# YiZhiXiaoGuLI/xerus

Measured on AMD Instinct MI355X. Metric: GFLOP/s on TT contraction + TT-round sweep time, order-10 rank-256, higher is better.
Workload: dtype f64; 1 GPU; TT order-10 n=20 rank-256: <x,y> + x.round(256) per step; order=10, mode_size=20, rank=256, parallelism=replicas x1

## Files before the change

### include/xerus_amd.h

```cpp
#ifndef XERUS_AMD_H
#define XERUS_AMD_H

#include <stddef.h>
#include <stdint.h>

#ifdef __cplusplus
extern "C" {
#endif

typedef struct xrs_handle_s* xrs_handle_t;

#define XRS_OK 0
#define XRS_EINVAL (-1)
#define XRS_ENOMEM (-2)
#define XRS_EHIP (-3)
#define XRS_ENUMERIC 1

int xrs_create(xrs_handle_t* handle, int device);
int xrs_destroy(xrs_handle_t handle);
int xrs_set_stream(xrs_handle_t handle, void* hip_stream);
void* xrs_get_stream(xrs_handle_t handle);
int xrs_synchronize(xrs_handle_t handle);
const char* xrs_last_error(void);
const char* xrs_version(void);

int xrs_malloc(xrs_handle_t handle, void** ptr, size_t bytes);
int xrs_free(xrs_handle_t handle, void* ptr);
size_t xrs_pool_bytes(xrs_handle_t handle);
int xrs_upload(xrs_handle_t handle, double* dst_dev, const double* src_host, size_t n);
int xrs_download(xrs_handle_t handle, double* dst_host, const double* src_dev, size_t n);
int xrs_memset_zero(xrs_handle_t handle, double* dst_dev, size_t n);
int xrs_copy(xrs_handle_t handle, double* dst_dev, const double* src_dev, size_t n);

int xrs_nrm2(xrs_handle_t handle, double* result, const double* x, size_t n);
int xrs_dot(xrs_handle_t handle, double* result, const double* x, const double* y, size_t n);
int xrs_asum(xrs_handle_t handle, double* result, const double* x, size_t n);
int xrs_scal(xrs_handle_t handle, double* x, double alpha, size_t n);
int xrs_axpy(xrs_handle_t handle, double* y, double alpha, const double* x, size_t n);
int xrs_scale_rows(xrs_handle_t handle, double* X, const double* s, size_t m, size_t n);

int xrs_gemm(xrs_handle_t handle, double* C, size_t M, size_t N, double alpha,
             const double* A, size_t lda, int transA, size_t K,
             const double* B, size_t ldb, int transB);

int xrs_gemm_batched(xrs_handle_t handle, size_t count, double* const* C, size_t M, size_t N, double alpha,
                     const double* const* A, size_t lda, int transA, size_t K,
                     const double* const* B, size_t ldb, int transB);

int xrs_gemm_sym(xrs_handle_t handle, double* C, size_t N, double alpha,
                 const double* A, size_t lda, int transA, size_t K,
                 const double* B, size_t ldb, int transB);

int xrs_gemm_forms(xrs_handle_t handle, size_t count, double* const* C, size_t M, size_t N, double alpha,
                   const double* const* A, size_t lda, int transA, size_t K,
                   const double* const* B, size_t ldb, int transB, int sym, int tri);

int xrs_gemm_f32(xrs_handle_t handle, float* C, size_t M, size_t N, float alpha,
                 const float* A, size_t lda, int transA, size_t K,
                 const float* B, size_t ldb, int transB);

int xrs_permute(xrs_handle_t handle, double* out, const double* in, size_t ndim,
                const size_t* dims, const size_t* shuffle);

int xrs_qc(xrs_handle_t handle, double* Q, double* C, size_t* rank, const double* A, size_t m, size_t n);
int xrs_cq(xrs_handle_t handle, double* C, double* Q, size_t* rank, const double* A, size_t m, size_t n);
int xrs_qr(xrs_handle_t handle, double* Q, double* R, const double* A, size_t m, size_t n);
int xrs_rq(xrs_handle_t handle, double* R, double* Q, const double* A, size_t m, size_t n);
int xrs_svd(xrs_handle_t handle, double* U, double* S, double* Vt, const double* A, size_t m, size_t n);
int xrs_svd_batched(xrs_handle_t handle, double* U, double* S, double* Vt, int* status,
                    const double* A, size_t batch, size_t m, size_t n);
int xrs_svd_batched_fits(size_t m, size_t n);
int xrs_solve(xrs_handle_t handle, double* X, const double* A, size_t m, size_t n, const double* B, size_t p);
int xrs_solve_least_squares(xrs_handle_t handle, double* X, const double* A, size_t m, size_t n, const double* B, size_t p);
int xrs_svd_rows_vt(xrs_handle_t handle, double* S, double* Vt, int* sweeps, const double* A, size_t p, size_t q, int kernel);
int xrs_sym_tridiag(xrs_handle_t handle, double* d, double* e, const double* A, size_t n);
int xrs_sym_eig_top(xrs_handle_t handle, double* lam, double* Ut, int* status, const double* A, size_t n, size_t kk);


int xrs_tt_move_core(xrs_handle_t handle, size_t d, const size_t* n, size_t* r, double** cores,
                     int canonicalized, size_t core_position, size_t position, int keep_rank);
int xrs_tt_round(xrs_handle_t handle, size_t d, const size_t* n, size_t* r, double** cores,
                 int canonicalized, size_t core_position, const size_t* max_ranks, double eps);
int xrs_tt_soft_threshold(xrs_handle_t handle, size_t d, const size_t* n, size_t* r, double** cores,
                          int canonicalized, size_t core_position, const double* taus);
int xrs_tt_entrywise_product(xrs_handle_t handle, size_t d, const size_t* ext, const size_t* ra, const double* const* A,
                             const size_t* rb, const double* const* B, double alpha, double** out);
int xrs_tt_entrywise_square(xrs_handle_t handle, size_t d, const size_t* ext, const size_t* r, const double* const* A,
                            double alpha, double** out, size_t* r_out);
// ... 60 lines not shown

int xrs_philox_words(xrs_handle_t handle, uint32_t* out, size_t s, size_t q, uint64_t seed, uint32_t stream);
int xrs_gaussian_matrix(xrs_handle_t handle, double* G, size_t s, size_t m, uint64_t seed, uint32_t stream);
#define XRS_SKETCH_FUSED 1
#define XRS_SKETCH_MATERIALISED 2
int xrs_sketch_gaussian(xrs_handle_t handle, double* Y, size_t s, const double* A, size_t m, size_t n, uint64_t seed,
                        uint32_t stream, int route);
int xrs_sketch_last_route(xrs_handle_t handle);


int xrs_als_local_apply(xrs_handle_t handle, double* y, const double* x, size_t rl, size_t n, size_t rr, size_t pl,
                        size_t pr, const double* L, const double* A, const double* R, int normal);
#define XRS_CG_CONVERGED 0
#define XRS_CG_MAX_ITER 1
#define XRS_CG_BREAKDOWN 2
int xrs_als_local_cg(xrs_handle_t handle, double* x, const double* b, size_t rl, size_t n, size_t rr, size_t pl,
                     size_t pr, const double* L, const double* A, const double* R, int normal, double tol,
                     size_t max_iter, size_t check_every, size_t* iters, double* relres, int* status);

#define XRS_EIG_CONVERGED 0
#define XRS_EIG_MAX_ITER 1
#define XRS_EIG_BREAKDOWN 2
int xrs_als_local_eig(xrs_handle_t handle, double* x, size_t rl, size_t n, size_t rr, size_t pl, size_t pr,
                      const double* L, const double* A, const double* R, double tol, size_t max_iter, size_t check_every,
                      double* theta, size_t* iters, double* relres, int* status);
int xrs_geneig_lowest(int k, const double* G, const double* H, double* theta, double* c);

#define XRS_KFAM_GEMM 1u
#define XRS_KFAM_PERMUTE 2u
#define XRS_KFAM_QR 4u
#define XRS_KFAM_SVD 8u
#define XRS_KFAM_ELEMWISE 16u
#define XRS_KFAM_SPLITK 32u
int xrs_prof_begin(xrs_handle_t handle, uint32_t family_mask);
int xrs_prof_end(xrs_handle_t handle, size_t* launches, double* total_ms, double* flops, double* bytes);

#ifdef __cplusplus
}
#endif
#endif
```

### xerus_amd/capi.py

```python
from __future__ import annotations

import ctypes as C
import os
from typing import Sequence

import numpy as np

_HERE = os.path.dirname(os.path.abspath(__file__))
LIB_PATH = os.environ.get("XRS_LIB_PATH") or os.path.join(_HERE, "libxerus_amd.so")

_SZ = C.c_size_t
_DP = C.c_void_p

SIGNATURES = {
    "xrs_create": (C.c_int, [C.POINTER(_DP), C.c_int]),
    "xrs_destroy": (C.c_int, [_DP]),
    "xrs_set_stream": (C.c_int, [_DP, _DP]),
    "xrs_get_stream": (_DP, [_DP]),
    "xrs_synchronize": (C.c_int, [_DP]),
    "xrs_last_error": (C.c_char_p, []),
    "xrs_version": (C.c_char_p, []),
    "xrs_malloc": (C.c_int, [_DP, C.POINTER(_DP), _SZ]),
    "xrs_free": (C.c_int, [_DP, _DP]),
    "xrs_pool_bytes": (_SZ, [_DP]),
    "xrs_upload": (C.c_int, [_DP, _DP, _DP, _SZ]),
    "xrs_download": (C.c_int, [_DP, _DP, _DP, _SZ]),
    "xrs_memset_zero": (C.c_int, [_DP, _DP, _SZ]),
    "xrs_copy": (C.c_int, [_DP, _DP, _DP, _SZ]),
    "xrs_nrm2": (C.c_int, [_DP, C.POINTER(C.c_double), _DP, _SZ]),
    "xrs_dot": (C.c_int, [_DP, C.POINTER(C.c_double), _DP, _DP, _SZ]),
    "xrs_asum": (C.c_int, [_DP, C.POINTER(C.c_double), _DP, _SZ]),
    "xrs_scal": (C.c_int, [_DP, _DP, C.c_double, _SZ]),
    "xrs_axpy": (C.c_int, [_DP, _DP, C.c_double, _DP, _SZ]),
    "xrs_scale_rows": (C.c_int, [_DP, _DP, _DP, _SZ, _SZ]),
    "xrs_gemm": (C.c_int, [_DP, _DP, _SZ, _SZ, C.c_double, _DP, _SZ, C.c_int, _SZ, _DP, _SZ, C.c_int]),
    "xrs_gemm_f32": (C.c_int, [_DP, _DP, _SZ, _SZ, C.c_float, _DP, _SZ, C.c_int, _SZ, _DP, _SZ, C.c_int]),
    "xrs_gemm_sym": (C.c_int,[_DP, _DP, _SZ, C.c_double, _DP, _SZ, C.c_int, _SZ, _DP, _SZ, C.c_int]),
    "xrs_gemm_batched": (C.c_int, [_DP, _SZ, C.POINTER(_DP), _SZ, _SZ, C.c_double, C.POINTER(_DP), _SZ, C.c_int, _SZ,
                                   C.POINTER(_DP), _SZ, C.c_int]),
    "xrs_gemm_forms": (C.c_int, [_DP, _SZ, C.POINTER(_DP), _SZ, _SZ, C.c_double, C.POINTER(_DP), _SZ, C.c_int, _SZ,
                                 C.POINTER(_DP), _SZ, C.c_int, C.c_int, C.c_int]),
    "xrs_permute": (C.c_int, [_DP, _DP, _DP, _SZ, C.POINTER(_SZ), C.POINTER(_SZ)]),
    "xrs_qc": (C.c_int, [_DP, _DP, _DP, C.POINTER(_SZ), _DP, _SZ, _SZ]),
    "xrs_cq": (C.c_int, [_DP, _DP, _DP, C.POINTER(_SZ), _DP, _SZ, _SZ]),
    "xrs_qr": (C.c_int, [_DP, _DP, _DP, _DP, _SZ, _SZ]),
    "xrs_rq": (C.c_int, [_DP, _DP, _DP, _DP, _SZ, _SZ]),
    "xrs_svd": (C.c_int, [_DP, _DP, _DP, _DP, _DP, _SZ, _SZ]),
    "xrs_svd_batched": (C.c_int, [_DP, _DP, _DP, _DP, C.POINTER(C.c_int), _DP, _SZ, _SZ, _SZ]),
    "xrs_svd_batched_fits": (C.c_int, [_SZ, _SZ]),
    "xrs_solve": (C.c_int, [_DP, _DP, _DP, _SZ, _SZ, _DP, _SZ]),
    "xrs_solve_least_squares": (C.c_int, [_DP, _DP, _DP, _SZ, _SZ, _DP, _SZ]),
    "xrs_svd_rows_vt": (C.c_int, [_DP, _DP, _DP, C.POINTER(C.c_int), _DP, _SZ, _SZ, C.c_int]),
    "xrs_sym_eig_top": (C.c_int, [_DP, _DP, _DP, C.POINTER(C.c_int), _DP, _SZ, _SZ]),
    "xrs_sym_tridiag": (C.c_int, [_DP, _DP, _DP, _DP, _SZ]),
    "xrs_tt_entrywise_product": (C.c_int, [_DP, _SZ, C.POINTER(_SZ), C.POINTER(_SZ), C.POINTER(_DP), C.POINTER(_SZ), C.POINTER(_DP),
                                           C.c_double, C.POINTER(_DP)]),
    "xrs_tt_entrywise_square": (C.c_int, [_DP, _SZ, C.POINTER(_SZ), C.POINTER(_SZ), C.POINTER(_DP), C.c_double, C.POINTER(_DP),
                                          C.POINTER(_SZ)]),
    "xrs_tt_rank_one_argmax": (C.c_int, [_DP, _SZ, C.POINTER(_SZ), C.POINTER(_DP), C.POINTER(_SZ)]),
    "xrs_tt_operator_apply": (C.c_int, [_DP, _SZ, C.POINTER(_SZ), C.POINTER(_SZ), C.POINTER(_SZ), C.POINTER(_SZ), C.POINTER(_DP),
                                        C.POINTER(_SZ), C.POINTER(_DP), C.c_int, C.POINTER(_DP)]),
    "xrs_tt_move_core": (C.c_int, [_DP, _SZ, C.POINTER(_SZ), C.POINTER(_SZ), C.POINTER(_DP), C.c_int, _SZ, _SZ, C.c_int]),
    "xrs_tt_round": (C.c_int, [_DP, _SZ, C.POINTER(_SZ), C.POINTER(_SZ), C.POINTER(_DP), C.c_int, _SZ,
                               C.POINTER(_SZ), C.c_double]),
    "xrs_tt_dot": (C.c_int, [_DP, C.POINTER(C.c_double), _SZ, C.POINTER(_SZ), C.POINTER(_SZ), C.POINTER(_DP),
                             C.POINTER(_SZ), C.POINTER(_DP)]),
    "xrs_tt_dot_async": (C.c_int, [_DP, _SZ, C.POINTER(_SZ), C.POINTER(_SZ), C.POINTER(_DP), C.POINTER(_SZ),
                                   C.POINTER(_DP)]),
    "xrs_tt_dot_wait": (C.c_int, [_DP, C.POINTER(C.c_double)]),
    "xrs_tt_dot_f32": (C.c_int, [_DP, C.POINTER(C.c_double), _SZ, C.POINTER(_SZ), C.POINTER(_SZ), C.POINTER(_DP),
                                 C.POINTER(_SZ), C.POINTER(_DP)]),
    "xrs_tt_round_sharded": (C.c_int, [_DP, _SZ, C.POINTER(_SZ), C.POINTER(_SZ), C.POINTER(_DP), C.POINTER(_SZ),
                                       C.c_double, _DP, _DP, C.POINTER(C.c_int)]),
    "xrs_tt_round_sharded_ex": (C.c_int, [_DP, _SZ, C.POINTER(_SZ), C.POINTER(_SZ), C.POINTER(_DP), C.POINTER(_SZ),
# ... 8 lines not shown
                                     C.POINTER(_DP), C.POINTER(_DP)]),
    "xrs_tt_last_round_path": (C.c_int, [_DP]),
    "xrs_tt_soft_threshold": (C.c_int, [_DP, _SZ, C.POINTER(_SZ), C.POINTER(_SZ), C.POINTER(_DP), C.c_int, _SZ,
                                        C.POINTER(C.c_double)]),
    "xrs_comm_unique_id": (C.c_int, [_DP]),
    "xrs_comm_create": (C.c_int, [_DP, C.c_int, C.c_int, _DP, C.POINTER(_DP)]),
    "xrs_comm_emulate": (C.c_int, [_DP, C.c_int, C.POINTER(_DP)]),
    "xrs_comm_destroy": (C.c_int, [_DP]),
    "xrs_comm_calls": (_SZ, [_DP]),
    "xrs_comm_allreduce": (C.c_int, [_DP, _DP, _SZ]),
    "xrs_comm_allgather": (C.c_int, [_DP, _DP, _DP, _SZ]),
    "xrs_tt_gather_sharded": (C.c_int, [_DP, _SZ, C.POINTER(_SZ), C.c_int, C.c_int, C.POINTER(_SZ), C.POINTER(_DP),
                                        C.POINTER(_DP), _DP, _DP]),
    "xrs_tt_shard": (C.c_int, [_DP, _SZ, C.POINTER(_SZ), C.c_int, C.c_int, C.POINTER(_SZ), C.POINTER(_DP), C.POINTER(_DP)]),
    "xrs_uq_basis": (C.c_int, [_DP, _DP, _DP, _SZ, _SZ]),
    "xrs_uq_stack_congruence": (C.c_int, [_DP, _DP, _DP, _DP, _DP, _SZ, _SZ, _SZ, _SZ]),
    "xrs_uq_quadform": (C.c_int, [_DP, C.POINTER(C.c_double), _DP, _DP, _SZ, _SZ]),
    "xrs_philox_words": (C.c_int, [_DP, _DP, _SZ, _SZ, C.c_uint64, C.c_uint32]),
    "xrs_gaussian_matrix": (C.c_int, [_DP, _DP, _SZ, _SZ, C.c_uint64, C.c_uint32]),
    "xrs_sketch_gaussian": (C.c_int, [_DP, _DP, _SZ, _DP, _SZ, _SZ, C.c_uint64, C.c_uint32, C.c_int]),
    "xrs_sketch_last_route": (C.c_int, [_DP]),
    "xrs_als_local_apply": (C.c_int, [_DP, _DP, _DP, _SZ, _SZ, _SZ, _SZ, _SZ, _DP, _DP, _DP, C.c_int]),
    "xrs_als_local_cg": (C.c_int, [_DP, _DP, _DP, _SZ, _SZ, _SZ, _SZ, _SZ, _DP, _DP, _DP, C.c_int, C.c_double, _SZ, _SZ,
                                   C.POINTER(_SZ), C.POINTER(C.c_double), C.POINTER(C.c_int)]),
    "xrs_als_local_eig": (C.c_int, [_DP, _DP, _SZ, _SZ, _SZ, _SZ, _SZ, _DP, _DP, _DP, C.c_double, _SZ, _SZ,
                                    C.POINTER(C.c_double), C.POINTER(_SZ), C.POINTER(C.c_double), C.POINTER(C.c_int)]),
    "xrs_geneig_lowest": (C.c_int, [C.c_int, C.POINTER(C.c_double), C.POINTER(C.c_double), C.POINTER(C.c_double),
                                    C.POINTER(C.c_double)]),
    "xrs_prof_begin": (C.c_int, [_DP, C.c_uint32]),
    "xrs_prof_end": (C.c_int, [_DP, C.POINTER(_SZ), C.POINTER(C.c_double), C.POINTER(C.c_double),
                               C.POINTER(C.c_double)]),
}

KFAM_GEMM, KFAM_PERMUTE, KFAM_QR, KFAM_SVD, KFAM_ELEMWISE, KFAM_SPLITK = 1, 2, 4, 8, 16, 32
ROUND_PATHS = {0: None, 1: "chain", 2: "truncate", 3: "reference", 4: "general"}
SKETCH_AUTO, SKETCH_FUSED, SKETCH_MATERIALISED = 0, 1, 2
SKETCH_ROUTES = {0: None, 1: "fused", 2: "materialised"}

_lib = None


class XrsError(RuntimeError):

    def __init__(self, fn: str, code: int, msg: str):
        super().__init__(f"{fn} failed with status {code}: {msg}")
        self.code = code


def load(path: str | None = None) -> C.CDLL:
    global _lib
    if _lib is not None and path is None:
        return _lib
    p = path or LIB_PATH
    if not os.path.exists(p):
        raise ImportError(f"{p} is missing: build it with `python -c 'import __graft_entry__ as g; g.build()'`")
    lib = C.CDLL(p)
    for name, (res, args) in SIGNATURES.items():
        f = getattr(lib, name)
        f.restype = res
        f.argtypes = args
    if path is None:
        _lib = lib
    return lib


def _check(fn: str, status: int):
    if status != 0:
# ... 63 lines not shown
        return DeviceArray(self, tuple(int(s) for s in shape))

    def zeros(self, shape) -> "DeviceArray":
        d = DeviceArray(self, tuple(int(s) for s in shape))
        _check("xrs_memset_zero", self.lib.xrs_memset_zero(self.h, _DP(d.ptr), d.size))
        return d

    def gemm(self, C_: "DeviceArray", M, N, alpha, A: "DeviceArray", lda, transA, K, B: "DeviceArray", ldb, transB):
        _check("xrs_gemm", self.lib.xrs_gemm(self.h, _DP(C_.ptr), M, N, alpha, _DP(A.ptr), lda, int(transA), K,
                                            _DP(B.ptr), ldb, int(transB)))

    def gemm_f32(self, C_: "Float32Array", M, N, alpha, A: "Float32Array", lda, transA, K, B: "Float32Array", ldb, transB):
        _check("xrs_gemm_f32", self.lib.xrs_gemm_f32(self.h, _DP(C_.ptr), M, N, float(alpha), _DP(A.ptr), lda, int(transA),
                                                    K, _DP(B.ptr), ldb, int(transB)))

    def array_f32(self, a: np.ndarray) -> "Float32Array":
        return Float32Array.from_host(self, a)

    def gemm_sym(self, C_: "DeviceArray", N, alpha, A: "DeviceArray", lda, transA, K, B: "DeviceArray", ldb, transB):
        _check("xrs_gemm_sym", self.lib.xrs_gemm_sym(self.h, _DP(C_.ptr), N, alpha, _DP(A.ptr), lda, int(transA), K,
                                                    _DP(B.ptr), ldb, int(transB)))

    def gemm_batched(self, Cs, M, N, alpha, As, lda, transA, K, Bs, ldb, transB):
        cnt = len(Cs)
        tab = lambda xs: (_DP * max(1, cnt))(*[_DP(x.ptr) for x in xs])
        _check("xrs_gemm_batched", self.lib.xrs_gemm_batched(self.h, cnt, tab(Cs), M, N, alpha, tab(As), lda, int(transA),
                                                            K, tab(Bs), ldb, int(transB)))

    def gemm_forms(self, Cs, M, N, alpha, As, lda, transA, K, Bs, ldb, transB, sym: bool = False, tri: int = 0):
        cnt = len(Cs)
        tab = lambda xs: (_DP * max(1, cnt))(*[_DP(x.ptr) for x in xs])
        _check("xrs_gemm_forms", self.lib.xrs_gemm_forms(self.h, cnt, tab(Cs), M, N, alpha, tab(As), lda, int(transA), K,
                                                        tab(Bs), ldb, int(transB), int(sym), int(tri)))

    def tangent_to_tt(self, n, r, Us, Vs, add_base: bool):
        d = len(n)
        tab = lambda xs: (_DP * d)(*[_DP(x.ptr) for x in xs])
        out = (_DP * d)()
        _check("xrs_tt_tangent_to_tt", self.lib.xrs_tt_tangent_to_tt(self.h, d, _arr(n), _arr(r), tab(Us), tab(Vs),
                                                                    int(add_base), out))
        cores = []
        for k in range(d):
            shape = (2 * r[k] if k else 1, n[k], 2 * r[k + 1] if k + 1 < d else 1)
            c = DeviceArray(self, shape, ptr=out[k])
            c.owned = True
            cores.append(c)
        return cores

    def matmul(self, A: "DeviceArray", transA: bool, B: "DeviceArray", transB: bool, alpha: float = 1.0):
        am, ak = (A.shape[1], A.shape[0]) if transA else (A.shape[0], A.shape[1])
        bk, bn = (B.shape[1], B.shape[0]) if transB else (B.shape[0], B.shape[1])
        assert ak == bk, (A.shape, B.shape)
        out = self.empty((am, bn))
        self.gemm(out, am, bn, alpha, A, A.shape[1], transA, ak, B, B.shape[1], transB)
        return out

    def permute(self, out: "DeviceArray", inp: "DeviceArray", dims, shuffle):
        _check("xrs_permute", self.lib.xrs_permute(self.h, _DP(out.ptr), _DP(inp.ptr), len(dims), _arr(dims),
                                                  _arr(shuffle)))

    def reshuffle(self, inp: "DeviceArray", shuffle):
        dims = inp.shape
        out_dims = [0] * len(dims)
        for i, s in enumerate(shuffle):
            out_dims[s] = dims[i]
        out = self.empty(tuple(out_dims))
# ... 486 lines not shown
```

### xerus_amd/csrc/elementwise.hpp

```cpp
#pragma once
#include <algorithm>

#include "runtime.hpp"

namespace xrs {

void reduce_to_device(xrs_handle_t h, int mode, const double* x, const double* y, size_t n, double* out_dev,
                      double* partial = nullptr);
double reduce_to_host(xrs_handle_t h, int mode, const double* x, const double* y, size_t n);
void scal(xrs_handle_t h, double* x, double alpha, size_t n);
void axpy(xrs_handle_t h, double* y, double alpha, const double* x, size_t n);
void ldexp_copy(xrs_handle_t h, double* dst, const double* src, int ex, size_t n);
constexpr int kAmaxMany = 64;
void amax_enqueue(xrs_handle_t h, const double* const* x, const size_t* n, int count, double* out_dev);
void norms_enqueue(xrs_handle_t h, const double* const* x, const size_t* n, int count, double* out_dev);
int range_exponent(double am);
int range_exponent(xrs_handle_t h, const double* A, size_t n);
void scale_rows(xrs_handle_t h, double* X, const double* s, size_t m, size_t n);
void scale_cols(xrs_handle_t h, double* X, const double* s, size_t m, size_t n);
void diag_sum(xrs_handle_t h, double* out, const double* X, size_t P, size_t m);
void offset_add(xrs_handle_t h, double* out, const size_t* out_dims, const double* in, const size_t* in_dims, size_t nd,
                const size_t* offsets, double alpha);
void strided_eval(xrs_handle_t h, double* out, const double* in, size_t nd, const size_t* out_dims, const size_t* in_strides,
                  size_t nt, const size_t* tr_dims, const size_t* tr_strides, size_t base);

constexpr int kTriA = 1, kTriB = 2;
void gemm(xrs_handle_t h, double* C, size_t M, size_t N, double alpha, const double* A, size_t lda, bool ta, size_t K,
          const double* B, size_t ldb, bool tb, int tri = 0);
constexpr int kGemmBatchMax = 32;
void gemm_batched(xrs_handle_t h, int count, double* const* C, size_t M, size_t N, double alpha, const double* const* A,
                  size_t lda, bool ta, size_t K, const double* const* B, size_t ldb, bool tb, bool sym = false,
                  int tri = 0);
void gemm_sym(xrs_handle_t h, double* C, size_t N, double alpha, const double* A, size_t lda, bool ta, size_t K,
              const double* B, size_t ldb, bool tb);

struct GemmSpec {
    const double* A;
    const double* B;
    double* C;
    size_t M, N, K, lda, ldb;
    bool ta, tb;
};
inline void gemm(xrs_handle_t h, const GemmSpec& g) {
    gemm(h, g.C, g.M, g.N, 1.0, g.A, g.lda, g.ta, g.K, g.B, g.ldb, g.tb);
}

void permute(xrs_handle_t h, double* out, const double* in, size_t ndim, const size_t* dims, const size_t* shuffle);

}
```

### xerus_amd/csrc/tt.hip

```cpp
#include <algorithm>
#include <atomic>
#include <chrono>
#include <condition_variable>
#include <limits>
#include <memory>
#include <mutex>
#include <thread>
#include <cstdio>
#include <cstdlib>
#include <cmath>
#include <string>
#include <vector>

#include "tt_common.hpp"

namespace xrs {

namespace ttd {


std::vector<size_t> maximal_ranks(const TT& t) {
    std::vector<size_t> rk(t.r + 1, t.r + t.d);
    size_t cur = 1;
    for (size_t i = 0; i + 1 < t.d; ++i) {
// ... 102 lines not shown
    }
    DevBuf S(h, g * 8), Vt(h, g * g * 8), st(h, 64);
    XRS_HIP(hipMemsetAsync(st.d(), 0, 64, h->stream));
    jacobi_right_vectors(h, F, int(g), wide, S.d(), Vt.d(), st.as<int>(), 60);
    jacobi_settle(h, st.as<int>(), int(g), int(g), [&](int kernel) {
        jacobi_vt(h, F, int(g), false, int(g), int(g), S.d(), Vt.d(), int(g), st.as<int>(), 60, kernel);
    });
    std::vector<double> s(g);
    XRS_HIP(hipMemcpyAsync(s.data(), S.d(), g * 8, hipMemcpyDeviceToHost, h->stream));
    host_wait(h);
    const size_t kk = svd_cut(s, max_rank, eps);
    double* T = t.alloc(m * kk);
    if (wide) gemm(h, T, m, kk, 1.0, F, g, false, g, Vt.d(), g, true);
    else gemm(h, T, m, kk, 1.0, t.core[k], nn, false, nn, Vt.d(), g, true);
    if (soft > 0.0) {
        hipLaunchKernelGGL(k_soft_cols, dim3(unsigned(std::min<size_t>((m * kk + 255) / 256, 4096))), dim3(256), 0, h->stream, T, S.d(), m, kk,
                           soft);
        check_launch("k_soft_cols");
    }
    double* cur = t.alloc(kk * nn);
    if (wide) gemm(h, cur, kk, nn, 1.0, Vt.d(), g, false, g, Q, nn, false);
    else XRS_HIP(hipMemcpyAsync(cur, Vt.d(), kk * nn * 8, hipMemcpyDeviceToDevice, h->stream));
    double* prv = t.alloc(prow * kk);
    gemm(h, prv, prow, kk, 1.0, t.core[k - 1], m, false, m, T, kk, false);
    t.release(T);
    t.release(F);
    t.release(Q);
    t.replace(k, cur);
    t.replace(k - 1, prv);
    t.r[k] = kk;
}


void left_gram_step(TT& t, std::vector<double*>& G, double* T, size_t k, bool do_reduce) {
    xrs_handle_t h = t.h;
    if (k == 0) {
        gemm_sym(h, G[1], t.r[1], 1.0, t.core[0], t.r[1], true, t.rows_left(0), t.core[0], t.r[1], false);
        if (do_reduce) t.reduce(G[1], t.r[1] * t.r[1]);
        return;
    }
    const size_t a = t.r[k], b = t.r[k + 1], cols = t.cols_right(k);
    gemm(h, T, a, cols, 1.0, G[k], a, false, a, t.core[k], cols, false);
    gemm_sym(h, G[k + 1], b, 1.0, t.core[k], b, true, a * t.n[k], T, b, false);
    if (do_reduce) t.reduce(G[k + 1], b * b);
}

void right_gram_step(TT& t, std::vector<double*>& H, double* T, size_t k, bool do_reduce) {
    xrs_handle_t h = t.h;
    const size_t last = t.d - 1;
    if (k == last) {
        const size_t cl = t.cols_right(last);
        gemm_sym(h, H[last], t.r[last], 1.0, t.core[last], cl, false, cl, t.core[last], cl, true);
        if (do_reduce) t.reduce(H[last], t.r[last] * t.r[last]);
        return;
    }
    const size_t a = t.r[k], b = t.r[k + 1], cols = t.cols_right(k);
    gemm(h, T, a * t.n[k], b, 1.0, t.core[k], b, false, b, H[k + 1], b, false);
    gemm_sym(h, H[k], a, 1.0, t.core[k], cols, false, cols, T, cols, true);
    if (do_reduce) t.reduce(H[k], a * a);
}

void gram_chains(TT& t, std::vector<double*>& G, std::vector<double*>& H, std::vector<DevBuf>& store, bool left) {
    const size_t d = t.d;
    xrs_handle_t h = t.h;
    G.assign(d, nullptr);
    H.assign(d, nullptr);
    size_t tmax = 1;
    for (size_t k = 1; k + 1 < d; ++k) tmax = std::max(tmax, t.size(k));
    DevBuf TL(h, tmax * 8), TR(h, tmax * 8);
    if (t.sharded()) {
        for (size_t s = 0; s + 1 < d; ++s) {
            const size_t kl = s + 1, kr = d - 1 - s;
            const size_t nl = left ? t.r[kl] * t.r[kl] : 0, nr = t.r[kr] * t.r[kr];
            store.emplace_back(h, (nl + nr) * 8);
            double* base = store.back().d();
            if (left) G[kl] = base;
            H[kr] = base + nl;
            if (left) {
                StreamFork fork(h);
                fork.side();
                left_gram_step(t, G, TL.d(), s, false);
                fork.main();
                right_gram_step(t, H, TR.d(), kr, false);
                fork.join();
            } else {
                right_gram_step(t, H, TR.d(), kr, false);
            }
            t.reduce(base, nl + nr);
        }
// ... 467 lines not shown
}

void soft_threshold(TT& t, bool canonicalized, size_t core_pos, const double* taus) {
    const size_t d = t.d;
    t.h->last_round_path = XRS_ROUND_REFERENCE;
    const size_t start = canonicalized ? core_pos : 0;
    for (size_t k = start; k + 1 < d; ++k) orth_right(t, k);
    for (size_t i = 0; i + 1 < d; ++i) truncate_edge(t, d - 1 - i, std::numeric_limits<size_t>::max(), 0.0, taus[i]);
}

double dot_two_ended(xrs_handle_t h, size_t d, const size_t* n, const size_t* rx, const double* const* X, const size_t* ry,
                     const double* const* Y, const TT* shard = nullptr) {
    const size_t m = d / 2;
    size_t emax = 1, tmax = 1;
    for (size_t k = 0; k <= d; ++k) emax = std::max(emax, rx[k] * ry[k]);
    for (size_t k = 0; k < d; ++k) tmax = std::max(tmax, std::max(ry[k] * n[k] * rx[k + 1], rx[k] * n[k] * ry[k + 1]));
    DevBuf P0(h, 2 * emax * 8), P1(h, 2 * emax * 8), TL(h, tmax * 8), TR(h, tmax * 8);
    const bool unit_l = rx[0] == 1 && ry[0] == 1, unit_r = rx[d] == 1 && ry[d] == 1;
    bool self = true;
    for (size_t k = 0; k < d && self; ++k) self = X[k] == Y[k] && rx[k + 1] == ry[k + 1];
    auto second = [&](const GemmSpec& g) {
        if (self) gemm_sym(h, g.C, g.M, 1.0, g.A, g.lda, g.ta, g.K, g.B, g.ldb, g.tb);
        else gemm(h, g);
    };
    if (!unit_l || !unit_r) {
        double* ones = scratch::host<double>(h, scratch::kHostDotOnes, 2);
        ones[0] = ones[1] = 1.0;
        XRS_HIP(hipMemcpyAsync(P0.d(), &ones[0], 8, hipMemcpyHostToDevice, h->stream));
        XRS_HIP(hipMemcpyAsync(P0.d() + emax, &ones[1], 8, hipMemcpyHostToDevice, h->stream));
    }
    struct EndStep {
        bool on = false, first = false;
        GemmSpec g1{}, g2{};
    };
    const size_t steps = std::max(m, d - m);
    auto plan = [&](size_t s, double* E, double* F, double* nb, EndStep& L, EndStep& R, size_t& ne) {
        L = EndStep{};
        R = EndStep{};
        ne = 0;
        if (s < m) {
            const size_t k = s, a = rx[k], b = ry[k], nk = n[k], a2 = rx[k + 1], b2 = ry[k + 1];
            L.on = true;
            L.first = !(s == 0 && unit_l);
            const double* T = L.first ? TL.d() : X[k];
            L.g1 = GemmSpec{E, X[k], TL.d(), b, nk * a2, a, b, nk * a2, true, false};
            L.g2 = GemmSpec{T, Y[k], nb, a2, b2, b * nk, a2, b2, true, false};
            ne = a2 * b2;
        }
        if (s < d - m) {
            const size_t k = d - 1 - s, a = rx[k], b = ry[k], nk = n[k], a2 = rx[k + 1], b2 = ry[k + 1];
            R.on = true;
            R.first = !(s == 0 && unit_r);
            const double* T = R.first ? TR.d() : X[k];
            R.g1 = GemmSpec{X[k], F, TR.d(), a * nk, b2, a2, a2, b2, false, false};
            R.g2 = GemmSpec{T, Y[k], nb + (shard ? ne : emax), a, b, nk * b2, nk * b2, nk * b2, false, true};
        }
    };
    double *E = P0.d(), *F = P0.d() + emax;
    double* nextbuf = P1.d();
    double* curbuf = P0.d();
    {
        StreamFork fork(h);
        for (size_t s = 0; s < steps; ++s) {
            EndStep L, R;
            size_t ne;
            plan(s, E, F, nextbuf, L, R, ne);
            if (L.on) {
                if (!shard) fork.side();
                if (L.first) gemm(h, L.g1);
                second(L.g2);
            }
            if (R.on) {
                if (!shard) fork.main();
                if (R.first) gemm(h, R.g1);
                second(R.g2);
            }
            if (shard) shard->reduce(nextbuf, ne + (R.on ? R.g2.M * R.g2.N : 0));
            if (L.on) E = L.g2.C;
            if (R.on) F = R.g2.C;
            std::swap(curbuf, nextbuf);
        }
        fork.join();
    }
    return reduce_to_host(h, 1, E, F, rx[m] * ry[m]);
}

double dot(xrs_handle_t h, size_t d, const size_t* n, const size_t* rx, const double* const* X, const size_t* ry,
           const double* const* Y, const TT* shard = nullptr) {
    size_t emax = 1, tmax = 1;
    for (size_t k = 0; k < d; ++k) {
        emax = std::max(emax, rx[k + 1] * ry[k + 1]);
        tmax = std::max(tmax, ry[k] * n[k] * rx[k + 1]);
    }
    if (d >= 4) return dot_two_ended(h, d, n, rx, X, ry, Y, shard);
    DevBuf E0(h, emax * 8), E1(h, emax * 8), T(h, tmax * 8);
    const double one = 1.0;
    XRS_HIP(hipMemcpyAsync(E0.d(), &one, 8, hipMemcpyHostToDevice, h->stream));
    double* E = E0.d();
    double* En = E1.d();
    for (size_t k = 0; k < d; ++k) {
        const size_t a = rx[k], b = ry[k], nk = n[k], a2 = rx[k + 1], b2 = ry[k + 1];
        gemm(h, T.d(), b, nk * a2, 1.0, E, b, true, a, X[k], nk * a2, false);
        gemm(h, En, a2, b2, 1.0, T.d(), a2, true, b * nk, Y[k], b2, false);
        if (shard) shard->reduce(En, a2 * b2);
        std::swap(E, En);
    }
    double* hs = scratch::host<double>(h, scratch::kHostResult);
    XRS_HIP(hipMemcpyAsync(hs, E, 8, hipMemcpyDeviceToHost, h->stream));
// ... 349 lines not shown
```

Before: 37630 GFLOP/s.

## Add fused thin-rank environment step kernel for TT dot and Gram sweeps

Adds MFMA-based HIP kernels that compute an environment step (S contracted with X and Y cores) in one launch when either the contracted ranks or the output ranks are small (≤32). Previously each such step took two GEMM calls plus a temporary. The new kernels are routed into the TT dot, left Gram and right Gram sweeps through flop and rank thresholds. They can also fold the first boundary Gram computation into the second step. Rank-256 interiors still use GEMMs, so only the low-rank boundary steps change, and the thin-output path adds atomic ticket-based cross-block reductions.

```diff
diff --git a/include/xerus_amd.h b/include/xerus_amd.h
--- a/include/xerus_amd.h
+++ b/include/xerus_amd.h
@@ -54,6 +54,9 @@
 int xrs_gemm_forms(xrs_handle_t handle, size_t count, double* const* C, size_t M, size_t N, double alpha,
                    const double* const* A, size_t lda, int transA, size_t K,
                    const double* const* B, size_t ldb, int transB, int sym, int tri);
+
+int xrs_env_step_thin(xrs_handle_t handle, double* out, const double* S, const double* X, const double* Y,
+                      size_t ax, size_t ay, size_t n, size_t bx, size_t by, int right, int sym);
 
 int xrs_gemm_f32(xrs_handle_t handle, float* C, size_t M, size_t N, float alpha,
                  const float* A, size_t lda, int transA, size_t K,
@@ -180,6 +183,7 @@
 #define XRS_KFAM_SVD 8u
 #define XRS_KFAM_ELEMWISE 16u
 #define XRS_KFAM_SPLITK 32u
+#define XRS_KFAM_THIN 64u
 int xrs_prof_begin(xrs_handle_t handle, uint32_t family_mask);
 int xrs_prof_end(xrs_handle_t handle, size_t* launches, double* total_ms, double* flops, double* bytes);
 
diff --git a/xerus_amd/capi.py b/xerus_amd/capi.py
--- a/xerus_amd/capi.py
+++ b/xerus_amd/capi.py
@@ -40,6 +40,7 @@
                                    C.POINTER(_DP), _SZ, C.c_int]),
     "xrs_gemm_forms": (C.c_int, [_DP, _SZ, C.POINTER(_DP), _SZ, _SZ, C.c_double, C.POINTER(_DP), _SZ, C.c_int, _SZ,
                                  C.POINTER(_DP), _SZ, C.c_int, C.c_int, C.c_int]),
+    "xrs_env_step_thin": (C.c_int, [_DP, _DP, _DP, _DP, _DP, _SZ, _SZ, _SZ, _SZ, _SZ, C.c_int, C.c_int]),
     "xrs_permute": (C.c_int, [_DP, _DP, _DP, _SZ, C.POINTER(_SZ), C.POINTER(_SZ)]),
     "xrs_qc": (C.c_int, [_DP, _DP, _DP, C.POINTER(_SZ), _DP, _SZ, _SZ]),
     "xrs_cq": (C.c_int, [_DP, _DP, _DP, C.POINTER(_SZ), _DP, _SZ, _SZ]),
@@ -114,7 +115,7 @@
                                C.POINTER(C.c_double)]),
 }
 
-KFAM_GEMM, KFAM_PERMUTE, KFAM_QR, KFAM_SVD, KFAM_ELEMWISE, KFAM_SPLITK = 1, 2, 4, 8, 16, 32
+KFAM_GEMM, KFAM_PERMUTE, KFAM_QR, KFAM_SVD, KFAM_ELEMWISE, KFAM_SPLITK, KFAM_THIN = 1, 2, 4, 8, 16, 32, 64
 ROUND_PATHS = {0: None, 1: "chain", 2: "truncate", 3: "reference", 4: "general"}
 SKETCH_AUTO, SKETCH_FUSED, SKETCH_MATERIALISED = 0, 1, 2
 SKETCH_ROUTES = {0: None, 1: "fused", 2: "materialised"}
@@ -244,6 +245,11 @@
         tab = lambda xs: (_DP * max(1, cnt))(*[_DP(x.ptr) for x in xs])
         _check("xrs_gemm_forms", self.lib.xrs_gemm_forms(self.h, cnt, tab(Cs), M, N, alpha, tab(As), lda, int(transA), K,
                                                         tab(Bs), ldb, int(transB), int(sym), int(tri)))
+
+    def env_step_thin(self, out: "DeviceArray", S: "DeviceArray", X: "DeviceArray", Y: "DeviceArray", ax, ay, n, bx, by,
+                      right: bool = False, sym: bool = False):
+        _check("xrs_env_step_thin", self.lib.xrs_env_step_thin(self.h, _DP(out.ptr), _DP(S.ptr), _DP(X.ptr), _DP(Y.ptr),
+                                                              ax, ay, n, bx, by, int(right), int(sym)))
 
     def tangent_to_tt(self, n, r, Us, Vs, add_base: bool):
         d = len(n)
diff --git a/xerus_amd/csrc/elementwise.hpp b/xerus_amd/csrc/elementwise.hpp
--- a/xerus_amd/csrc/elementwise.hpp
+++ b/xerus_amd/csrc/elementwise.hpp
@@ -45,6 +45,17 @@
     gemm(h, g.C, g.M, g.N, 1.0, g.A, g.lda, g.ta, g.K, g.B, g.ldb, g.tb);
 }
 
+constexpr int kThinNone = 0, kThinInput = 1, kThinOutput = 2;
+int env_thin_form(size_t ax, size_t ay, size_t n, size_t bx, size_t by);
+int env_thin_route(size_t ax, size_t ay, size_t n, size_t bx, size_t by, bool right);
+struct ThinFold {
+    const double* core;
+    size_t n0;
+    double* gram;
+};
+void env_step_thin(xrs_handle_t h, double* out, const double* S, const double* X, const double* Y, size_t ax, size_t ay,
+                   size_t n, size_t bx, size_t by, bool right, bool sym, const ThinFold* fold = nullptr);
+
 void permute(xrs_handle_t h, double* out, const double* in, size_t ndim, const size_t* dims, const size_t* shuffle);
 
 }
diff --git a/xerus_amd/csrc/env_thin.hip b/xerus_amd/csrc/env_thin.hip
--- /dev/null
+++ b/xerus_amd/csrc/env_thin.hip
@@ -0,0 +1,372 @@
+#include <algorithm>
+#include <cstdlib>
+
+#include <hip/hip_ext.h>
+
+#include "elementwise.hpp"
+#include "runtime.hpp"
+
+namespace xrs {
+
+typedef double d4 __attribute__((ext_vector_type(4)));
+
+namespace {
+
+struct ThinArgs {
+    double* out;
+    const double* S;
+    const double* X;
+    const double* Y;
+    int ax, ay, n, bx, by;
+    long sxp, sxi, sxu;
+    long syq, syi, syv;
+    int sym;
+    const double* c0;
+    int n0;
+    long c0j, c0p;
+    double* gram;
+    double* slab1;
+    double* slab2;
+    int* tickets;
+};
+
+constexpr int kFrag = 16 * 64;
+
+__device__ __forceinline__ double ld0(const double* __restrict__ p, long idx, bool ok) {
+    const double v = p[ok ? idx : 0];
+    return ok ? v : 0.0;
+}
+
+__device__ __forceinline__ void store_frag(const ThinArgs& a, const d4& f, int u0, int v0, int lane) {
+    const int lr = lane & 15, lk = lane >> 4;
+#pragma unroll
+    for (int r = 0; r < 4; ++r) {
+        const int u = u0 + lk + 4 * r, v = v0 + lr;
+        if (u >= a.bx || v >= a.by) continue;
+        if (!a.sym) {
+            a.out[size_t(u) * a.by + v] = f[r];
+        } else if (u >= v) {
+            a.out[size_t(u) * a.by + v] = f[r];
+            a.out[size_t(v) * a.by + u] = f[r];
+        }
+    }
+}
+
+template <int NK>
+__global__ void __launch_bounds__(256) k_env_step_thin_in(const ThinArgs a) {
+    constexpr int TM = NK > 4 ? 2 : 1;
+    __shared__ double red[3][4][64];
+    const int u0 = int(blockIdx.x) * 16, v0 = int(blockIdx.y) * 16;
+    if (a.sym && blockIdx.x < blockIdx.y) return;
+    const int lane = threadIdx.x & 63, w = threadIdx.x >> 6;
+    const int lr = lane & 15, lk = lane >> 4;
+    auto prow = [](int m) { return m < 4 * NK ? (m & 3) * NK + (m >> 2) : 1 << 20; };
+    double sA[TM][NK];
+    if (a.c0 != nullptr) {
+#pragma unroll
+        for (int tm = 0; tm < TM; ++tm)
+#pragma unroll
+            for (int ks = 0; ks < NK; ++ks) sA[tm][ks] = 0.0;
+        for (int j = 0; j < a.n0; ++j) {
+            double cp[TM], cq[NK];
+#pragma unroll
+            for (int tm = 0; tm < TM; ++tm) cp[tm] = ld0(a.c0, j * a.c0j + prow(16 * tm + lr) * a.c0p, prow(16 * tm + lr) < a.ax);
+#pragma unroll
+            for (int ks = 0; ks < NK; ++ks) cq[ks] = ld0(a.c0, j * a.c0j + (lk * NK + ks) * a.c0p, lk * NK + ks < a.ay);
+#pragma unroll
+            for (int tm = 0; tm < TM; ++tm)
+#pragma unroll
+                for (int ks = 0; ks < NK; ++ks) sA[tm][ks] = fma(cp[tm], cq[ks], sA[tm][ks]);
+        }
+        if (blockIdx.x == 0 && blockIdx.y == 0 && w == 0) {
+#pragma unroll
+            for (int tm = 0; tm < TM; ++tm)
+#pragma unroll
+                for (int ks = 0; ks < NK; ++ks) {
+                    const int p = prow(16 * tm + lr), q = lk * NK + ks;
+                    if (p < a.ax && q < a.ay) a.gram[size_t(p) * a.ay + q] = sA[tm][ks];
+                }
+        }
+    } else {
+#pragma unroll
+        for (int tm = 0; tm < TM; ++tm)
+#pragma unroll
+            for (int ks = 0; ks < NK; ++ks) {
+                const int p = prow(16 * tm + lr), q = lk * NK + ks;
+                sA[tm][ks] = ld0(a.S, long(p) * a.ay + q, p < a.ax && q < a.ay);
+            }
+    }
+    auto load = [&](int i, double (&yB)[NK], double (&xA)[NK]) {
+        const int ic = i < a.n ? i : a.n - 1;
+        const double* __restrict__ Yi = a.Y + ic * a.syi;
+        const double* __restrict__ Xi = a.X + ic * a.sxi;
+#pragma unroll
+        for (int ks = 0; ks < NK; ++ks) {
+            const int k = lk * NK + ks;
+            yB[ks] = ld0(Yi, k * a.syq + (v0 + lr) * a.syv, k < a.ay && v0 + lr < a.by);
+            xA[ks] = ld0(Xi, k * a.sxp + (u0 + lr) * a.sxu, k < a.ax && u0 + lr < a.bx);
+        }
+    };
+    d4 acc = {0.0, 0.0, 0.0, 0.0};
+    double yB[NK], xA[NK];
+    load(w, yB, xA);
+    for (int i = w; i < a.n; i += 4) {
+        double yN[NK], xN[NK];
+        load(i + 4, yN, xN);
+        d4 Z[TM];
+#pragma unroll
+        for (int tm = 0; tm < TM; ++tm) {
+            Z[tm] = d4{0.0, 0.0, 0.0, 0.0};
+#pragma unroll
+            for (int ks = 0; ks < NK; ++ks) Z[tm] = __builtin_amdgcn_mfma_f64_16x16x4f64(sA[tm][ks], yB[ks], Z[tm], 0, 0, 0);
+        }
+#pragma unroll
+        for (int ks = 0; ks < NK; ++ks) acc = __builtin_amdgcn_mfma_f64_16x16x4f64(xA[ks], Z[ks >> 2][ks & 3], acc, 0, 0, 0);
+#pragma unroll
+        for (int ks = 0; ks < NK; ++ks) {
+            yB[ks] = yN[ks];
+            xA[ks] = xN[ks];
+        }
+    }
+    if (w > 0) {
+#pragma unroll
+        for (int r = 0; r < 4; ++r) red[w - 1][r][lane] = acc[r];
+    }
+    __syncthreads();
+    if (w > 0) return;
+#pragma unroll
+    for (int g = 0; g < 3; ++g)
+#pragma unroll
+        for (int r = 0; r < 4; ++r) acc[r] += red[g][r][lane];
+    store_frag(a, acc, u0, v0, lane);
+}
+
+__device__ __forceinline__ bool last_arriver(int* ticket, int count, int* flag) {
+    asm volatile("s_waitcnt vmcnt(0)" ::: "memory");
+    __syncthreads();
+    if (threadIdx.x == 0) {
+        const int t = __hip_atomic_fetch_add(ticket, 1, __ATOMIC_RELAXED, __HIP_MEMORY_SCOPE_AGENT);
+        if (t == count - 1) __hip_atomic_store(ticket, 0, __ATOMIC_RELAXED, __HIP_MEMORY_SCOPE_AGENT);
+        *flag = t == count - 1;
+    }
+    __syncthreads();
+    return *flag != 0;
+}
+
+__device__ __forceinline__ void put_partial(double* slab, int tile, const d4& f, int lane) {
+#pragma unroll
+    for (int r = 0; r < 4; ++r)
+        __hip_atomic_store(&slab[(tile * 4 + r) * 64 + lane], f[r], __ATOMIC_RELAXED, __HIP_MEMORY_SCOPE_AGENT);
+}
+__device__ __forceinline__ d4 sum_partials(const double* slab, int count, int tile, int lane) {
+    d4 s = {0.0, 0.0, 0.0, 0.0};
+    for (int c0 = 0; c0 < count; c0 += 16) {
+        double v[16][4];
+#pragma unroll
+        for (int j = 0; j < 16; ++j) {
+            const int c = c0 + j < count ? c0 + j : 0;
+#pragma unroll
+            for (int r = 0; r < 4; ++r)
+                v[j][r] = __hip_atomic_load(&slab[size_t(c) * kFrag + (tile * 4 + r) * 64 + lane], __ATOMIC_RELAXED,
+                                            __HIP_MEMORY_SCOPE_AGENT);
+        }
+#pragma unroll
+        for (int j = 0; j < 16; ++j)
+            if (c0 + j < count)
+#pragma unroll
+                for (int r = 0; r < 4; ++r) s[r] += v[j][r];
+    }
+    return s;
+}
+
+__global__ void __launch_bounds__(256) k_env_step_thin_out(const ThinArgs a) {
+    __shared__ double red[4][16][64];
+    __shared__ double Ss[64][33], Ys[32][33];
+    __shared__ int flag;
+    const int tid = threadIdx.x, lane = tid & 63, w = tid >> 6;
+    const int lr = lane & 15, lk = lane >> 4;
+    const int i = blockIdx.y;
+    const int prow0 = int(blockIdx.x) * 64;
+    const int pb = prow0 + 16 * w;
+    const double* __restrict__ Yi = a.Y + i * a.syi;
+    const double* __restrict__ Xi = a.X + i * a.sxi;
+    const bool two = a.by > 16;
+    const bool ycont = a.syv == 1;
+    auto fetch = [&](int q0, double (&sv)[8], double (&yv)[4]) {
+#pragma unroll
+        for (int j = 0; j < 8; ++j) {
+            const int e = tid + 256 * j, p = prow0 + (e >> 5), q = q0 + (e & 31);
+            sv[j] = ld0(a.S, long(p) * a.ay + q, p < a.ax && q < a.ay);
+        }
+#pragma unroll
+        for (int j = 0; j < 4; ++j) {
+            const int e = tid + 256 * j, q = q0 + (ycont ? e >> 5 : e & 31), v = ycont ? e & 31 : e >> 5;
+            yv[j] = ld0(Yi, q * a.syq + v * a.syv, q < a.ay && v < a.by);
+        }
+    };
+    d4 W[2] = {};
+    double sv[8], yv[4];
+    fetch(0, sv, yv);
+    for (int q0 = 0; q0 < a.ay; q0 += 32) {
+        __syncthreads();
+#pragma unroll
+        for (int j = 0; j < 8; ++j) Ss[(tid + 256 * j) >> 5][(tid + 256 * j) & 31] = sv[j];
+#pragma unroll
+        for (int j = 0; j < 4; ++j) {
+            const int e = tid + 256 * j;
+            Ys[ycont ? e >> 5 : e & 31][ycont ? e & 31 : e >> 5] = yv[j];
+        }
+        __syncthreads();
+        fetch(q0 + 32, sv, yv);
+#pragma unroll
+        for (int j = 0; j < 8; ++j) {
+            const double sa = Ss[16 * w + lr][4 * j + lk];
+            W[0] = __builtin_amdgcn_mfma_f64_16x16x4f64(sa, Ys[4 * j + lk][lr], W[0], 0, 0, 0);
+            if (two) W[1] = __builtin_amdgcn_mfma_f64_16x16x4f64(sa, Ys[4 * j + lk][16 + lr], W[1], 0, 0, 0);
+        }
+    }
+    d4 o[2][2] = {};
+#pragma unroll
+    for (int tu = 0; tu < 2; ++tu) {
+        double xa[4];
+#pragma unroll
+        for (int r = 0; r < 4; ++r) {
+            const int p = pb + 4 * r + lk, u = 16 * tu + lr;
+            xa[r] = ld0(Xi, p * a.sxp + u * a.sxu, p < a.ax && u < a.bx);
+        }
+        if (16 * tu < a.bx)
+#pragma unroll
+            for (int r = 0; r < 4; ++r) {
+                o[tu][0] = __builtin_amdgcn_mfma_f64_16x16x4f64(xa[r], W[0][r], o[tu][0], 0, 0, 0);
+                if (two) o[tu][1] = __builtin_amdgcn_mfma_f64_16x16x4f64(xa[r], W[1][r], o[tu][1], 0, 0, 0);
+            }
+    }
+#pragma unroll
+    for (int t = 0; t < 4; ++t)
+#pragma unroll
+        for (int r = 0; r < 4; ++r) red[w][t * 4 + r][lane] = o[t >> 1][t & 1][r];
+    __syncthreads();
+    d4 s = {0.0, 0.0, 0.0, 0.0};
+#pragma unroll
+    for (int g = 0; g < 4; ++g)
+#pragma unroll
+        for (int r = 0; r < 4; ++r) s[r] += red[g][w * 4 + r][lane];
+    const int blocks = int(gridDim.x);
+    if (blocks > 1) {
+        put_partial(a.slab1 + (size_t(i) * blocks + blockIdx.x) * kFrag, w, s, lane);
+        if (!last_arriver(&a.tickets[i], blocks, &flag)) return;
+        s = sum_partials(a.slab1 + size_t(i) * blocks * kFrag, blocks, w, lane);
+    }
+    if (a.n > 1) {
+        put_partial(a.slab2 + size_t(i) * kFrag, w, s, lane);
+        if (!last_arriver(&a.tickets[a.n], a.n, &flag)) return;
+        s = sum_partials(a.slab2, a.n, w, lane);
+    }
+    store_frag(a, s, 16 * (w >> 1), 16 * (w & 1), lane);
+}
+
+constexpr double kThinMaxFlops = 1.5e8, kThinMaxFlopsRight = 6e7;
+constexpr size_t kThinMaxRankRight = 24, kThinOutMaxRank = 64;
+
+double thin_flops(size_t ax, size_t ay, size_t n, size_t bx, size_t by) {
+    return 2.0 * double(n) * (double(ax) * double(ay) * double(by) + double(ax) * double(bx) * double(by));
+}
+
+template <int NK>
+void launch_in(xrs_handle_t h, const ThinArgs& a, dim3 grid, hipEvent_t start, hipEvent_t stop) {
+    hipExtLaunchKernelGGL(k_env_step_thin_in<NK>, grid, dim3(256), 0, h->stream, start, stop, 0, a);
+}
+
+}
+
+int env_thin_form(size_t ax, size_t ay, size_t n, size_t bx, size_t by) {
+    if (ax == 0 || ay == 0 || n == 0 || bx == 0 || by == 0) return kThinNone;
+    const size_t big = size_t(1) << 30;
+    if (ax >= big || ay >= big || bx >= big || by >= big || n >= big) return kThinNone;
+    if (ax <= 32 && ay <= 32 && (bx + 15) / 16 <= 65535 && (by + 15) / 16 <= 65535) return kThinInput;
+    if (bx <= 32 && by <= 32 && n + 1 <= size_t(xrs_handle_s::kTicketCap)) return kThinOutput;
+    return kThinNone;
+}
+
+int env_thin_route(size_t ax, size_t ay, size_t n, size_t bx, size_t by, bool right) {
+    const char* e = std::getenv("XRS_THIN_STEP");
+    if (e && e[0] == '0') return kThinNone;
+    const int form = env_thin_form(ax, ay, n, bx, by);
+    const double flops = thin_flops(ax, ay, n, bx, by);
+    const size_t in = std::max(ax, ay);
+    if (form == kThinInput) return (right ? flops <= kThinMaxFlopsRight && in <= kThinMaxRankRight : flops <= kThinMaxFlops) ? form : kThinNone;
+    if (form == kThinOutput) return in <= kThinOutMaxRank ? form : kThinNone;
+    return kThinNone;
+}
+
+void env_step_thin(xrs_handle_t h, double* out, const double* S, const double* X, const double* Y, size_t ax, size_t ay,
+                   size_t n, size_t bx, size_t by, bool right, bool sym, const ThinFold* fold) {
+    const int form = env_thin_form(ax, ay, n, bx, by);
+    XRS_REQUIRE(form != kThinNone, "neither the contracted nor the output ranks are <= 32");
+    XRS_REQUIRE(!sym || (ax == ay && bx == by && X == Y), "a symmetric step needs X = Y");
+    XRS_REQUIRE(!fold || (sym && form == kThinInput), "only a symmetric thin-input step folds the first Gram in");
+    ThinArgs a{};
+    a.out = out;
+    a.S = S;
+    a.X = X;
+    a.Y = Y;
+    a.ax = int(ax), a.ay = int(ay), a.n = int(n), a.bx = int(bx), a.by = int(by);
+    if (!right) {
+        a.sxp = long(n * bx), a.sxi = long(bx), a.sxu = 1;
+        a.syq = long(n * by), a.syi = long(by), a.syv = 1;
+    } else {
+        a.sxp = 1, a.sxi = long(ax), a.sxu = long(n * ax);
+        a.syq = 1, a.syi = long(ay), a.syv = long(n * ay);
+    }
+    a.sym = sym ? 1 : 0;
+    if (fold) {
+        a.c0 = fold->core;
+        a.n0 = int(fold->n0);
+        a.c0j = right ? 1 : long(ax);
+        a.c0p = right ? long(fold->n0) : 1;
+        a.gram = fold->gram;
+    }
+    const double flops = thin_flops(ax, ay, n, bx, by);
+    const double bytes = 8.0 * (double(ax) * ay + double(n) * (double(ax) * bx + double(ay) * by) + double(bx) * by);
+    if (form == kThinInput) {
+        const dim3 grid(unsigned((bx + 15) / 16), unsigned((by + 15) / 16));
+        KernelTimer timer(h, XRS_KFAM_THIN, flops, bytes, true);
+        switch ((std::max(ax, ay) + 3) / 4) {
+            case 1: launch_in<1>(h, a, grid, timer.start(), timer.stop()); break;
+            case 2: launch_in<2>(h, a, grid, timer.start(), timer.stop()); break;
+            case 3: launch_in<3>(h, a, grid, timer.start(), timer.stop()); break;
+            case 4: launch_in<4>(h, a, grid, timer.start(), timer.stop()); break;
+            case 5: launch_in<5>(h, a, grid, timer.start(), timer.stop()); break;
+            case 6: launch_in<6>(h, a, grid, timer.start(), timer.stop()); break;
+            case 7: launch_in<7>(h, a, grid, timer.start(), timer.stop()); break;
+            default: launch_in<8>(h, a, grid, timer.start(), timer.stop()); break;
+        }
+        check_launch("k_env_step_thin_in");
+        return;
+    }
+    const size_t blocks = (ax + 63) / 64;
+    DevBuf slab(h, (n * blocks + n) * size_t(kFrag) * 8);
+    a.slab1 = slab.d();
+    a.slab2 = slab.d() + n * blocks * size_t(kFrag);
+    a.tickets = h->tickets;
+    KernelTimer timer(h, XRS_KFAM_THIN, flops, bytes, true);
+    hipExtLaunchKernelGGL(k_env_step_thin_out, dim3(unsigned(blocks), unsigned(n)), dim3(256), 0, h->stream, timer.start(),
+                          timer.stop(), 0, a);
+    check_launch("k_env_step_thin_out");
+}
+
+}
+
+extern "C" int xrs_env_step_thin(xrs_handle_t h, double* out, const double* S, const double* X, const double* Y, size_t ax,
+                                 size_t ay, size_t n, size_t bx, size_t by, int right, int sym) {
+    return xrs::guarded([&] {
+        XRS_REQUIRE(h, "null handle");
+        XRS_REQUIRE(out && S && X && Y, "null pointer");
+        XRS_REQUIRE(ax && ay && n && bx && by, "a rank or the mode size is 0");
+        XRS_REQUIRE(out != S && out != X && out != Y, "out must not alias an operand");
+        XRS_REQUIRE(xrs::env_thin_form(ax, ay, n, bx, by) != xrs::kThinNone,
+                    "neither the contracted ranks (ax, ay) nor the output ranks (bx, by) are <= 32");
+        xrs::fence_readers(h);
+        xrs::env_step_thin(h, out, S, X, Y, ax, ay, n, bx, by, right != 0, sym != 0);
+    });
+}
diff --git a/xerus_amd/csrc/tt.hip b/xerus_amd/csrc/tt.hip
--- a/xerus_amd/csrc/tt.hip
+++ b/xerus_amd/csrc/tt.hip
@@ -158,14 +158,30 @@
 }
 
 
+constexpr size_t kFoldMaxCore = 4096;
+static bool fold_first(const TT& t, bool right) {
+    if (t.sharded() || t.d < 3) return false;
+    const size_t e = right ? t.d - 1 : 0, s = right ? t.d - 2 : 1;
+    const size_t in = right ? t.r[t.d - 1] : t.r[1], out = right ? t.r[t.d - 2] : t.r[2];
+    return t.size(e) <= kFoldMaxCore && env_thin_route(in, in, t.n[s], out, out, right) == kThinInput;
+}
+
 void left_gram_step(TT& t, std::vector<double*>& G, double* T, size_t k, bool do_reduce) {
     xrs_handle_t h = t.h;
     if (k == 0) {
+        if (fold_first(t, false)) return;
         gemm_sym(h, G[1], t.r[1], 1.0, t.core[0], t.r[1], true, t.rows_left(0), t.core[0], t.r[1], false);
         if (do_reduce) t.reduce(G[1], t.r[1] * t.r[1]);
         return;
     }
     const size_t a = t.r[k], b = t.r[k + 1], cols = t.cols_right(k);
+    if (env_thin_route(a, a, t.n[k], b, b, false) != kThinNone) {
+        const ThinFold first{t.core[0], t.n[0], G[1]};
+        env_step_thin(h, G[k + 1], G[k], t.core[k], t.core[k], a, a, t.n[k], b, b, false, true,
+                      k == 1 && fold_first(t, false) ? &first : nullptr);
+        if (do_reduce) t.reduce(G[k + 1], b * b);
+        return;
+    }
     gemm(h, T, a, cols, 1.0, G[k], a, false, a, t.core[k], cols, false);
     gemm_sym(h, G[k + 1], b, 1.0, t.core[k], b, true, a * t.n[k], T, b, false);
     if (do_reduce) t.reduce(G[k + 1], b * b);
@@ -175,12 +191,20 @@
     xrs_handle_t h = t.h;
     const size_t last = t.d - 1;
     if (k == last) {
+        if (fold_first(t, true)) return;
         const size_t cl = t.cols_right(last);
         gemm_sym(h, H[last], t.r[last], 1.0, t.core[last], cl, false, cl, t.core[last], cl, true);
         if (do_reduce) t.reduce(H[last], t.r[last] * t.r[last]);
         return;
     }
     const size_t a = t.r[k], b = t.r[k + 1], cols = t.cols_right(k);
+    if (env_thin_route(b, b, t.n[k], a, a, true) != kThinNone) {
+        const ThinFold first{t.core[last], t.n[last], H[last]};
+        env_step_thin(h, H[k], H[k + 1], t.core[k], t.core[k], b, b, t.n[k], a, a, true, true,
+                      k + 1 == last && fold_first(t, true) ? &first : nullptr);
+        if (do_reduce) t.reduce(H[k], a * a);
+        return;
+    }
     gemm(h, T, a * t.n[k], b, 1.0, t.core[k], b, false, b, H[k + 1], b, false);
     gemm_sym(h, H[k], a, 1.0, t.core[k], cols, false, cols, T, cols, true);
     if (do_reduce) t.reduce(H[k], a * a);
@@ -714,6 +738,8 @@
     struct EndStep {
         bool on = false, first = false;
         GemmSpec g1{}, g2{};
+        int thin = kThinNone;
+        size_t ca = 0, cb = 0, nk = 0, oa = 0, ob = 0;
     };
     const size_t steps = std::max(m, d - m);
     auto plan = [&](size_t s, double* E, double* F, double* nb, EndStep& L, EndStep& R, size_t& ne) {
@@ -727,6 +753,8 @@
             const double* T = L.first ? TL.d() : X[k];
             L.g1 = GemmSpec{E, X[k], TL.d(), b, nk * a2, a, b, nk * a2, true, false};
             L.g2 = GemmSpec{T, Y[k], nb, a2, b2, b * nk, a2, b2, true, false};
+            L.ca = a, L.cb = b, L.nk = nk, L.oa = a2, L.ob = b2;
+            L.thin = L.first ? env_thin_route(a, b, nk, a2, b2, false) : kThinNone;
             ne = a2 * b2;
         }
         if (s < d - m) {
@@ -736,6 +764,8 @@
             const double* T = R.first ? TR.d() : X[k];
             R.g1 = GemmSpec{X[k], F, TR.d(), a * nk, b2, a2, a2, b2, false, false};
             R.g2 = GemmSpec{T, Y[k], nb + (shard ? ne : emax), a, b, nk * b2, nk * b2, nk * b2, false, true};
+            R.ca = a2, R.cb = b2, R.nk = nk, R.oa = a, R.ob = b;
+            R.thin = R.first ? env_thin_route(a2, b2, nk, a, b, true) : kThinNone;
         }
     };
     double *E = P0.d(), *F = P0.d() + emax;
@@ -749,13 +779,19 @@
             plan(s, E, F, nextbuf, L, R, ne);
             if (L.on) {
                 if (!shard) fork.side();
-                if (L.first) gemm(h, L.g1);
-                second(L.g2);
+                if (L.thin) env_step_thin(h, L.g2.C, E, L.g1.B, L.g2.B, L.ca, L.cb, L.nk, L.oa, L.ob, false, self);
+                else {
+                    if (L.first) gemm(h, L.g1);
+                    second(L.g2);
+                }
             }
             if (R.on) {
                 if (!shard) fork.main();
-                if (R.first) gemm(h, R.g1);
-                second(R.g2);
+                if (R.thin) env_step_thin(h, R.g2.C, F, R.g1.A, R.g2.B, R.ca, R.cb, R.nk, R.oa, R.ob, true, self);
+                else {
+                    if (R.first) gemm(h, R.g1);
+                    second(R.g2);
+                }
             }
             if (shard) shard->reduce(nextbuf, ne + (R.on ? R.g2.M * R.g2.N : 0));
             if (L.on) E = L.g2.C;
```

Result: no change. 38290 GFLOP/s, median of 3 (+1.8%).
